# microsoft/NOTSOFAR1-Challenge

Hardware: AMD Instinct MI355X
Metric: CSS real-time-factor (sep. audio sec/wall sec) on 7-ch 16 kHz (higher is better)
Workload: dtype f32 (float32 operands on v_mfma_f32_32x32x2_f32 in every Linear layer, attention product and transform: the reference's own operand precision; MVDR covariance / solve f64)

## Files before the change

notsofar1-challenge_amd/csrc/gemm_f32.hip:

```cpp
#include <algorithm>
#include <type_traits>

#include "gemm_common.hpp"

namespace css {

namespace {

constexpr int F_BK = 16;
constexpr int F_LD = 20;
constexpr int F_BUF = (128 + BN) * F_LD;
constexpr int F_PATCH_LD = 36;

typedef float f32x4 __attribute__((ext_vector_type(4)));

__device__ __forceinline__ float epi_value(float acc, float bn, float bm, int act, bool has_res, float rv, float alpha) {
    float v = acc + bn + bm;
    if (act == ACT_RELU) v = fmaxf(v, 0.f);
    else if (act == ACT_SIGMOID) v = sigmoidf_(v);
    if (has_res) v = rv + alpha * v;
    return v;
}

template <int TM, bool BD, bool FAST>
__device__ __forceinline__ void f32_tile(const GemmArgs& g, const float* __restrict__ A, const float* __restrict__ B,
                                         float* __restrict__ C, const int m0, const int n0, float* __restrict__ lds) {
    const int tid = threadIdx.x, lane = tid & 63, w = tid >> 6, c = lane & 31, h = lane >> 5;
    const int M = g.M, N = g.N;
    constexpr int BM = 32 * TM;
    constexpr int NPA = (BM + 63) / 64;
    const int srow = tid >> 2, sk = (tid & 3) * 4;
    const int64_t extA = (int64_t)(M - 1) * g.lda + (g.lda > g.K ? g.lda : g.K), extB = (int64_t)(N - 1) * g.ldb + (g.ldb > g.K ? g.ldb : g.K);
    const __amdgpu_buffer_rsrc_t rsA = __builtin_amdgcn_make_buffer_rsrc(const_cast<float*>(A), 0, (int)(extA * 4), 0x00020000);
    const __amdgpu_buffer_rsrc_t rsB = __builtin_amdgcn_make_buffer_rsrc(const_cast<float*>(B), 0, (int)((BD ? (int64_t)((N + 31) / 32 * 32) * g.K : extB) * 4), 0x00020000);
    const int voA = (int)(((int64_t)(m0 + srow) * g.lda + sk) * 4), voB = (int)(((int64_t)(n0 + srow) * g.ldb + sk) * 4);
    const int passA = (int)(64 * g.lda * 4), passB = (int)(64 * g.ldb * 4);
    const bool a1_on = (BM % 64 == 0) || srow < BM % 64;
#ifndef F32_TOOLS
#define F32_TOOLS 0
#endif
#ifndef F32_PROBE
#define F32_PROBE 0
#endif
#ifndef F32_FAST_EPILOGUE
#define F32_FAST_EPILOGUE 1
#endif
#ifndef F32_SPREAD
#define F32_SPREAD 1
#endif
#ifndef F32_TRANSPOSED
#define F32_TRANSPOSED 0
#endif
#ifndef F32_STORE_GUARD
#define F32_STORE_GUARD 1
#endif
#if F32_STORE_GUARD
#define F32_AFTER_STORE(o) asm volatile("s_nop 0" : : "v"(o));
#else
#define F32_AFTER_STORE(o)
#endif
#ifndef F32_DMA
#define F32_DMA 0
#endif
#if F32_DMA
    constexpr int D_BUF = (128 + BN) * 16;
    const int dseg = ((tid & 3) ^ ((tid >> 4) & 3)) * 4;
    const int dvoA = (int)(((int64_t)(m0 + srow) * g.lda + dseg) * 4), dvoB = (int)(((int64_t)(n0 + srow) * g.ldb + dseg) * 4);
    const bool a1_wave = (BM % 64 == 0) || w < (BM % 64) / 16;
    typedef __attribute__((address_space(3))) void lds_void;
#define F32_GLOAD(k0, buf)                                                                                       \
    _Pragma("unroll") for (int i = 0; i < NPA; ++i) {                                                            \
        if (i + 1 < NPA || a1_wave)                                                                              \
            __builtin_amdgcn_raw_ptr_buffer_load_lds(rsA, (lds_void*)(lds + (buf) * D_BUF + (i * 64 + 16 * w) * 16), 16, dvoA, (k0) * 4 + i * passA, 0, 0); \
    }                                                                                                            \
    _Pragma("unroll") for (int i = 0; i < 2; ++i)                                                                \
        __builtin_amdgcn_raw_ptr_buffer_load_lds(rsB, (lds_void*)(lds + (buf) * D_BUF + (128 + i * 64 + 16 * w) * 16), 16, dvoB, (k0) * 4 + i * passB, 0, 0);
#define F32_LSTORE(buf) __builtin_amdgcn_s_waitcnt(0x0F70);
#define F32_GLOAD1(k0, j)
#undef F32_SPREAD
#define F32_SPREAD 0
#else
    f32x4 ra[NPA], rb[2];
    f32x4 wc[2], wn[2];
    const int vw = (int)((((int64_t)(n0 / 32 + w) * (g.K / 8)) * 64 + lane) * 16);
#define F32_GLOAD(k0, buf)                                                                                       \
    _Pragma("unroll") for (int i = 0; i < NPA; ++i) {                                                            \
        if (i + 1 < NPA || a1_on) ra[i] = __builtin_bit_cast(f32x4, __builtin_amdgcn_raw_buffer_load_b128(rsA, voA, (k0) * 4 + i * passA, 0)); \
    }                                                                                                            \
    if constexpr (!BD) {                                                                                         \
        _Pragma("unroll") for (int i = 0; i < 2; ++i)                                                            \
            rb[i] = __builtin_bit_cast(f32x4, __builtin_amdgcn_raw_buffer_load_b128(rsB, voB, (k0) * 4 + i * passB, 0)); \
    } else {                                                                                                     \
        wn[0] = __builtin_bit_cast(f32x4, __builtin_amdgcn_raw_buffer_load_b128(rsB, vw, ((k0) / 8) * 1024, 0)); \
        wn[1] = __builtin_bit_cast(f32x4, __builtin_amdgcn_raw_buffer_load_b128(rsB, vw, ((k0) / 8 + 1) * 1024, 0)); \
    }
#define F32_GLOAD1(k0, j)                                                                                        \
    {                                                                                                            \
        if ((j) < NPA) {                                                                                         \
            if ((j) + 1 < NPA || a1_on) ra[(j) < NPA ? (j) : 0] = __builtin_bit_cast(f32x4, __builtin_amdgcn_raw_buffer_load_b128(rsA, voA, (k0) * 4 + (j) * passA, 0)); \
        } else if ((j) < NPA + 2) {                                                                              \
            if constexpr (!BD) rb[(j) - NPA] = __builtin_bit_cast(f32x4, __builtin_amdgcn_raw_buffer_load_b128(rsB, voB, (k0) * 4 + ((j) - NPA) * passB, 0)); \
            else wn[(j) - NPA] = __builtin_bit_cast(f32x4, __builtin_amdgcn_raw_buffer_load_b128(rsB, vw, ((k0) / 8 + (j) - NPA) * 1024, 0)); \
        }                                                                                                        \
    }
#define F32_LSTORE(buf)                                                                                          \
    {                                                                                                            \
        float* as_ = lds + (buf) * F_BUF + srow * F_LD + sk;                                                     \
        _Pragma("unroll") for (int i = 0; i < NPA; ++i) {                                                        \
            if (i + 1 < NPA || a1_on) *reinterpret_cast<f32x4*>(as_ + i * 64 * F_LD) = ra[i];                    \
        }                                                                                                        \
        if constexpr (!BD) {                                                                                     \
            _Pragma("unroll") for (int i = 0; i < 2; ++i) *reinterpret_cast<f32x4*>(as_ + (128 + i * 64) * F_LD) = rb[i]; \
        }                                                                                                        \
    }
#endif
    f32x16 acc[TM];
#pragma unroll
    for (int i = 0; i < TM; ++i) acc[i] = f32x16{0};
    const int nk = g.K / F_BK;
#if F32_PROBE
    const unsigned long long t_in_ = (w == 0) ? __builtin_readcyclecounter() : 0;
#endif
    F32_GLOAD(0, 0)
    F32_LSTORE(0)
    if constexpr (BD) { wc[0] = wn[0]; wc[1] = wn[1]; }
    __syncthreads();
#if F32_DMA
    constexpr int S_BUF = D_BUF, S_LD = 16;
    const int sw4 = ((c >> 2) & 3) * 4;
    const int aoff = c * 16, boff = (128 + 32 * w + c) * 16;
#define F32_SLOT(ch) (((8 * (ch) + 4 * h)) ^ sw4)
#else
    constexpr int S_BUF = F_BUF, S_LD = F_LD;
    const int aoff = c * F_LD + 4 * h, boff = (128 + 32 * w + c) * F_LD + 4 * h;
#define F32_SLOT(ch) (8 * (ch))
#endif
    const float* __restrict__ bias = g.bias;
    const float* __restrict__ res = g.residual;
    const int act = g.act;
    const bool bias_m = bias && g.bias_along_m, bias_n = bias && !g.bias_along_m, has_res = res != nullptr;
    const int64_t ldc = g.ldc, ldr = g.ldr;
    const float alpha = g.alpha;
    const bool wide = FAST || ((ldc % 4 == 0) && (N % 4 == 0) && ((reinterpret_cast<uintptr_t>(C) & 15) == 0) &&
                               (!has_res || ((ldr % 4 == 0) && ((reinterpret_cast<uintptr_t>(res) & 15) == 0))));
    constexpr bool fast = FAST;
    const __amdgpu_buffer_rsrc_t rsC = __builtin_amdgcn_make_buffer_rsrc(C, 0, fast ? (int)((int64_t)M * ldc * 4) : 0, 0x00020000);
    const __amdgpu_buffer_rsrc_t rsR = __builtin_amdgcn_make_buffer_rsrc(const_cast<float*>(res), 0, (fast && has_res) ? (int)((int64_t)M * ldr * 4) : 0, 0x00020000);
    f32x4 rv[2][4];
#if F32_TRANSPOSED
    auto prefetch_fast = [&](int i, int slot, int lane_) {
        const int vo_ = (int)((((int64_t)m0 + (lane_ & 31)) * ldr + n0 + 32 * w + 4 * (lane_ >> 5)) * 4);
#pragma unroll
        for (int q = 0; q < 4; ++q)
            rv[slot][q] = __builtin_bit_cast(f32x4, __builtin_amdgcn_raw_buffer_load_b128(rsR, vo_, (int)((32 * i * ldr + 8 * q) * 4), 0));
    };
#else
    auto prefetch_fast = [&](int i, int slot, int lane_) {
        const int vo_ = (int)(((unsigned)(m0 + (lane_ >> 3)) * (unsigned)ldr + n0 + 32 * w + (lane_ & 7) * 4) * 4u);
#pragma unroll
        for (int j = 0; j < 4; ++j)
            rv[slot][j] = __builtin_bit_cast(f32x4, __builtin_amdgcn_raw_buffer_load_b128(rsR, vo_, (int)((unsigned)(32 * i + 8 * j) * (unsigned)ldr * 4u), 0));
    };
#endif
    auto prefetch = [&](int i, int slot, int lane_) {
        const int n_ = n0 + 32 * w + (lane_ & 7) * 4;
#pragma unroll
        for (int j = 0; j < 4; ++j) {
            const int m = m0 + 32 * i + (lane_ >> 3) + 8 * j;
            const int mc = m < M ? m : M - 1;
            rv[slot][j] = f32x4{0.f, 0.f, 0.f, 0.f};
            if (has_res && n_ < N) {
                if (wide) {
                    rv[slot][j] = *reinterpret_cast<const f32x4*>(res + (int64_t)mc * ldr + n_);
                } else {
#pragma unroll
                    for (int e = 0; e < 4; ++e) rv[slot][j][e] = res[(int64_t)mc * ldr + (n_ + e < N ? n_ + e : N - 1)];
                }
            }
        }
    };
#ifndef F32_ABLATE
#define F32_ABLATE 0
#endif
    f32x4 abl_a = {1.f, 2.f, 3.f, (float)lane}, abl_b = {0.5f, 0.25f, (float)w, 1.f};
#define F32_COMPUTE(buf)                                                                                         \
    {                                                                                                            \
        const float* as = lds + (buf) * S_BUF + aoff;                                                            \
        const float* bs = lds + (buf) * S_BUF + boff;                                                            \
        _Pragma("unroll") for (int ch = 0; ch < 2; ++ch) {                                                       \
            f32x4 b = abl_b;                                                                                     \
            if constexpr (BD) b = wc[ch];                                                                        \
            else if (!(F32_ABLATE & 4)) b = *reinterpret_cast<const f32x4*>(bs + F32_SLOT(ch));                  \
            f32x4 a[TM];                                                                                         \
            _Pragma("unroll") for (int i = 0; i < TM; ++i) {                                                     \
                a[i] = abl_a;                                                                                    \
                if (!(F32_ABLATE & 4)) a[i] = *reinterpret_cast<const f32x4*>(as + i * 32 * S_LD + F32_SLOT(ch)); \
            }                                                                                                    \
            __builtin_amdgcn_sched_barrier(0);                                                                   \
            _Pragma("unroll") for (int e = 0; e < 4; ++e) {                                                      \
                if (F32_SPREAD && spread_k0 >= 0 && !(e & 1)) { F32_GLOAD1(spread_k0, ch * 2 + (e >> 1)) __builtin_amdgcn_sched_barrier(0); } \
                _Pragma("unroll") for (int i = 0; i < TM; ++i) {                                                 \
                    if (F32_ABLATE & 8) asm volatile("v_mfma_f32_32x32x2_f32 %0, %1, %2, %0" : "+a"(acc[i]) : "v"(a[i][e]), "v"(b[e])); \
                    else if (F32_TRANSPOSED) acc[i] = __builtin_amdgcn_mfma_f32_32x32x2f32(b[e], a[i][e], acc[i], 0, 0, 0); \
                    else acc[i] = __builtin_amdgcn_mfma_f32_32x32x2f32(a[i][e], b[e], acc[i], 0, 0, 0);          \
                }                                                                                                \
                if (F32_SPREAD && spread_k0 >= 0) __builtin_amdgcn_sched_barrier(0);                             \
            }                                                                                                    \
            __builtin_amdgcn_sched_barrier(0);                                                                   \
        }                                                                                                        \
    }
#if F32_PROBE
    const bool probe = w == 0 && g.narrow_epilogue == 77 && g.range_flag;
    unsigned long long pc_ = 0, pl_ = 0, pb_ = 0, pt_ = 0;
    const unsigned long long t_loop_ = probe ? __builtin_readcyclecounter() : 0;
#define F32_CLK(var) if (probe) var = __builtin_readcyclecounter();
#else
#define F32_CLK(var)
#endif
    int spread_k0 = -1;
    for (int kt = 0; kt + 1 < nk; ++kt) {
#if F32_PROBE
        unsigned long long t0_ = 0, t1_ = 0, t2_ = 0, t3_ = 0;
#endif
        F32_CLK(t0_)
        if (F32_SPREAD) spread_k0 = (kt + 1) * F_BK;
        else if (!(F32_ABLATE & 2)) { F32_GLOAD((kt + 1) * F_BK, (kt + 1) & 1) }
        __builtin_amdgcn_sched_barrier(0);
        F32_COMPUTE(kt & 1)
        F32_CLK(t1_)
        if (!(F32_ABLATE & 2)) { F32_LSTORE((kt + 1) & 1) }
        if constexpr (BD) { wc[0] = wn[0]; wc[1] = wn[1]; }
        F32_CLK(t2_)
        if (!(F32_ABLATE & 1)) __syncthreads();
        F32_CLK(t3_)
#if F32_PROBE
        pc_ += t1_ - t0_; pl_ += t2_ - t1_; pb_ += t3_ - t2_; pt_ += 1;
#endif
    }
#if F32_PROBE
    if (probe && lane == 0) {
        unsigned long long* pr = reinterpret_cast<unsigned long long*>(g.range_flag) + 4096 + 4 * blockIdx.x;
        atomicAdd(pr + 0, pc_); atomicAdd(pr + 1, pl_); atomicAdd(pr + 2, pb_); atomicAdd(pr + 3, pt_);
        atomicAdd(pr + 4096 + 0, t_loop_ - t_in_);
        atomicAdd(pr + 4096 + 1, 1ull);
    }
    const unsigned long long t_out_ = probe ? __builtin_readcyclecounter() : 0;
#define F32_EPILOGUE_PROBE                                                                                       \
    if (probe && lane == 0) {                                                                                    \
        unsigned long long* pr = reinterpret_cast<unsigned long long*>(g.range_flag) + 4096 + 4 * blockIdx.x;    \
        atomicAdd(pr + 4096 + 2, __builtin_readcyclecounter() - t_out_);        \
    }
#else
#define F32_EPILOGUE_PROBE
#endif
#undef F32_CLK
    {
        int lane_ = lane;
        asm volatile("" : "+v"(lane_));
        if (fast) { if (has_res) prefetch_fast(0, 0, lane_); }
        else prefetch(0, 0, lane_);
    }
    spread_k0 = -1;
    F32_COMPUTE((nk - 1) & 1)
    __syncthreads();
#undef F32_COMPUTE
#undef F32_SLOT
#undef F32_GLOAD
#undef F32_GLOAD1
#undef F32_LSTORE

    int lane_e = lane;
    asm volatile("" : "+v"(lane_e));
    float* patch = lds + w * (32 * F_PATCH_LD);
    const int col4 = (lane_e & 7) * 4, n = n0 + 32 * w + col4, erow = lane_e >> 3;
    const bool col_ok = n < N;
    float bn[4] = {0.f, 0.f, 0.f, 0.f};
    if (bias_n) {
#pragma unroll
        for (int e = 0; e < 4; ++e) bn[e] = bias[n + e < N ? n + e : N - 1];
    }
#if F32_TRANSPOSED
    if (fast) {
        const int ce = lane_e & 31, he = lane_e >> 5, nw = n0 + 32 * w + 4 * he;
        const int voC = (int)((((int64_t)m0 + ce) * ldc + nw) * 4);
        const bool relu = act == ACT_RELU;
        f32x4 bq[4];
#pragma unroll
        for (int q = 0; q < 4; ++q) {
            bq[q] = f32x4{0.f, 0.f, 0.f, 0.f};
            if (bias_n) {
#pragma unroll
                for (int e = 0; e < 4; ++e) bq[q][e] = bias[nw + 8 * q + e];
            }
        }
#pragma unroll
        for (int i = 0; i < TM; ++i) {
            if (i + 1 < TM && has_res) prefetch_fast(i + 1, (i + 1) & 1, lane_e);
#pragma unroll
            for (int q = 0; q < 4; ++q) {
                f32x4 o;
#pragma unroll
                for (int e = 0; e < 4; ++e) {
                    float t = acc[i][4 * q + e] + bq[q][e];
                    if (relu) t = fmaxf(t, 0.f);
                    if (has_res) t = rv[i & 1][q][e] + alpha * t;
                    o[e] = t;
                }
                typedef unsigned int u32x4 __attribute__((ext_vector_type(4)));
                __builtin_amdgcn_raw_buffer_store_b128(__builtin_bit_cast(u32x4, o), rsC, voC, (int)((32 * i * ldc + 8 * q) * 4), 0);
                F32_AFTER_STORE(o)
#if F32_TRANSPOSED >= 2
                __builtin_amdgcn_sched_barrier(0);
                asm volatile("s_nop 7");
#if F32_TRANSPOSED >= 3
                asm volatile("s_nop 7");
#endif
                __builtin_amdgcn_sched_barrier(0);
#endif
            }
        }
        F32_EPILOGUE_PROBE
        return;
    }
#else
    if constexpr (FAST) {
        const int voC = (int)(((unsigned)(m0 + erow) * (unsigned)ldc + n) * 4u);
        auto epilogue = [&](auto relu_c, auto res_c) {
            const bool relu = relu_c;
            constexpr bool res = decltype(res_c)::value;
#pragma unroll
            for (int i = 0; i < TM; ++i) {
#pragma unroll
                for (int r = 0; r < 16; ++r) patch[((r & 3) + 8 * (r >> 2) + 4 * h) * F_PATCH_LD + c] = acc[i][r];
                if (i + 1 < TM && res) prefetch_fast(i + 1, (i + 1) & 1, lane_e);
#pragma unroll
                for (int j = 0; j < 4; ++j) {
                    const f32x4 v = *reinterpret_cast<const f32x4*>(patch + (erow + 8 * j) * F_PATCH_LD + col4);
                    f32x4 o;
#pragma unroll
                    for (int e = 0; e < 4; ++e) {
                        float t = v[e] + bn[e];
                        if (relu) t = fmaxf(t, 0.f);
                        if (res) t = rv[i & 1][j][e] + alpha * t;
                        o[e] = t;
                    }
                    typedef unsigned int u32x4 __attribute__((ext_vector_type(4)));
                    __builtin_amdgcn_raw_buffer_store_b128(__builtin_bit_cast(u32x4, o), rsC, voC, (int)((unsigned)(32 * i + 8 * j) * (unsigned)ldc * 4u), 0);
                    F32_AFTER_STORE(o)
                }
            }
        };
        if (has_res) epilogue(act == ACT_RELU, std::true_type{});
        else if (act == ACT_RELU) epilogue(std::true_type{}, std::false_type{});
        else epilogue(std::false_type{}, std::false_type{});
        F32_EPILOGUE_PROBE
        return;
    }
#endif
#pragma unroll
    for (int i = 0; i < TM; ++i) {
#if F32_TRANSPOSED
#pragma unroll
        for (int q = 0; q < 4; ++q)
            *reinterpret_cast<f32x4*>(patch + c * F_PATCH_LD + 8 * q + 4 * h) = f32x4{acc[i][4 * q], acc[i][4 * q + 1], acc[i][4 * q + 2], acc[i][4 * q + 3]};
#else
#pragma unroll
        for (int r = 0; r < 16; ++r) patch[((r & 3) + 8 * (r >> 2) + 4 * h) * F_PATCH_LD + c] = acc[i][r];
#endif
        if (i + 1 < TM) prefetch(i + 1, (i + 1) & 1, lane_e);
#pragma unroll
        for (int j = 0; j < 4; ++j) {
            const int row = erow + 8 * j, m = m0 + 32 * i + row;
            const f32x4 v = *reinterpret_cast<const f32x4*>(patch + row * F_PATCH_LD + col4);
            if (m >= M || !col_ok) continue;
            float* dst = C + (int64_t)m * ldc + n;
            const float bm = bias_m ? bias[m] : 0.f;
            f32x4 o;
#pragma unroll
            for (int e = 0; e < 4; ++e) o[e] = epi_value(v[e], bn[e], bm, act, has_res, rv[i & 1][j][e], alpha);
            if (wide) {
                *reinterpret_cast<f32x4*>(dst) = o;
            } else {
#pragma unroll
                for (int e = 0; e < 4; ++e)
                    if (n + e < N) dst[e] = o[e];
            }
        }
    }
    F32_EPILOGUE_PROBE
#undef F32_EPILOGUE_PROBE
}

}

struct F32Plan {
    int u, tiles_n, ncu, max_tm; int64_t U;
#if F32_TOOLS
    unsigned long long* dbg;
#endif
};

template <bool BD, bool FAST>
__global__ __launch_bounds__(256, 4) void gemm_f32_kernel(GemmArgs g, F32Plan p) {
    __shared__ __attribute__((aligned(16))) float lds[2 * F_BUF];
    const int b = blockIdx.x, v = b % p.ncu, j = b / p.ncu;
    const int64_t lo = p.U * v / p.ncu, hi = p.U * (v + 1) / p.ncu;
    int64_t pos = lo + (hi - lo) * j / 4;
    const int64_t end = lo + (hi - lo) * (j + 1) / 4;
    int want = std::min(1 + (b + j) % 4, p.max_tm);
    bool first = true;
#if F32_TOOLS
    if (p.dbg && threadIdx.x == 0) {
        p.dbg[4 * b + 0] = wall_clock64();
        p.dbg[4 * b + 2] = ((unsigned long long)__builtin_amdgcn_s_getreg(63508) << 32) | (unsigned)__builtin_amdgcn_s_getreg(63492);
        p.dbg[4 * b + 3] = __builtin_readcyclecounter();
    }
#endif
    const int64_t panel0 = pos / p.u;
    int r = (int)(pos - panel0 * p.u);
    int bz = (int)(panel0 / p.tiles_n), tn = (int)(panel0 - (int64_t)bz * p.tiles_n);
    while (pos < end) {
        const int tm = (int)std::min<int64_t>(std::min<int64_t>(want, end - pos), p.u - r);
        const float* A = g.A + (int64_t)bz * g.strideA;
        const float* B = g.B + (int64_t)bz * g.strideB;
        float* C = g.C + (int64_t)bz * g.strideC;
        if (!first) __syncthreads();
        first = false;
        switch (tm) {
            case 1: f32_tile<1, BD, FAST>(g, A, B, C, 32 * r, tn * BN, lds); break;
            case 2: f32_tile<2, BD, FAST>(g, A, B, C, 32 * r, tn * BN, lds); break;
            case 3: f32_tile<3, BD, FAST>(g, A, B, C, 32 * r, tn * BN, lds); break;
            default: f32_tile<4, BD, FAST>(g, A, B, C, 32 * r, tn * BN, lds); break;
        }
        pos += tm;
        want = p.max_tm;
        r += tm;
        if (r == p.u) {
            r = 0;
            if (++tn == p.tiles_n) { tn = 0; ++bz; }
        }
    }
#if F32_TOOLS
    if (p.dbg && threadIdx.x == 0) { p.dbg[4 * b + 1] = wall_clock64(); p.dbg[4 * b + 3] = __builtin_readcyclecounter() - p.dbg[4 * b + 3]; }
#endif
}

static bool f32_fast_epilogue(const GemmArgs& g) {
    const int64_t lim = (int64_t)1 << 31;
    const bool has_res = g.residual != nullptr;
    const bool wide = (g.ldc % 4 == 0) && (g.N % 4 == 0) && ((reinterpret_cast<uintptr_t>(g.C) & 15) == 0) &&
                      (g.batch == 1 || g.strideC % 4 == 0) &&
                      (!has_res || ((g.ldr % 4 == 0) && ((reinterpret_cast<uintptr_t>(g.residual) & 15) == 0)));
    return F32_FAST_EPILOGUE && wide && !(g.bias && g.bias_along_m) && (g.N % BN == 0) && g.act != ACT_SIGMOID &&
           (int64_t)g.M * g.ldc * 4 < lim && (!has_res || (int64_t)g.M * g.ldr * 4 < lim);
}

bool launch_gemm_f32(const GemmArgs& g, hipStream_t s, int forced_tm) {
    if (g.M <= 0 || g.N <= 0 || g.batch <= 0) return true;
    if (g.K <= 0 || g.K % F_BK) return false;
    const int64_t lim = (int64_t)1 << 31;
    if ((((int64_t)g.M + 128) * g.lda + g.K) * 4 >= lim || (((int64_t)g.N + 128) * g.ldb + g.K) * 4 >= lim) return false;
    if (g.b_frag32 && (g.N % 32 || g.K % 16 || g.batch != 1 || ((int64_t)g.N * g.K * 4 >= lim))) return false;
    if ((g.lda % 4) || (!g.b_frag32 && (g.ldb % 4)) || (reinterpret_cast<uintptr_t>(g.A) & 15) || (reinterpret_cast<uintptr_t>(g.B) & 15)) return false;
    constexpr int NCU = 256;
    F32Plan p;
    p.u = (g.M + 31) / 32;
    p.tiles_n = (g.N + BN - 1) / BN;
    p.ncu = NCU;
    p.max_tm = (forced_tm >= 1 && forced_tm <= 4) ? forced_tm : 4;
    p.U = (int64_t)p.u * p.tiles_n * g.batch;
#if F32_TOOLS
    p.dbg = g.narrow_epilogue == 77 ? reinterpret_cast<unsigned long long*>(g.range_flag) : nullptr;
#endif
    const bool fast = f32_fast_epilogue(g);
    void (*kern)(GemmArgs, F32Plan) = g.b_frag32 ? (fast ? gemm_f32_kernel<true, true> : gemm_f32_kernel<true, false>)
                                                 : (fast ? gemm_f32_kernel<false, true> : gemm_f32_kernel<false, false>);
    hipLaunchKernelGGL(kern, dim3(4 * NCU), dim3(256), 0, s, g, p);
    return true;
}


__global__ void f32_fragments_kernel(const float* __restrict__ src, int64_t ld_src, float* __restrict__ dst, int N, int K) {
    const int64_t idx = (int64_t)blockIdx.x * blockDim.x + threadIdx.x;
    const int64_t total = (int64_t)(N / 32) * (K / 8) * 64;
    if (idx >= total) return;
    const int lane = (int)(idx & 63);
    const int64_t t = idx >> 6;
    const int kc = (int)(t % (K / 8)), j = (int)(t / (K / 8));
    const float* p = src + (int64_t)(32 * j + (lane & 31)) * ld_src + 8 * kc + 4 * (lane >> 5);
    reinterpret_cast<float4*>(dst)[idx] = make_float4(p[0], p[1], p[2], p[3]);
}
void launch_f32_fragments(const float* src, int64_t ld_src, float* dst, int N, int K, hipStream_t s) {
    const int64_t total = (int64_t)(N / 32) * (K / 8) * 64;
    if (total <= 0) return;
    hipLaunchKernelGGL(f32_fragments_kernel, dim3((unsigned)((total + 255) / 256)), dim3(256), 0, s, src, ld_src, dst, N, K);
}

}
```

Baseline: 7340.

## Use deeper K slabs for fragment-weight f32 GEMM tiles with small TM

Adds a K-depth template parameter so the weights-as-fragments f32 GEMM path stages 32- or 64-wide K slabs of A in LDS for TM 1-3 tiles, instead of 16. This cuts the number of syncthreads and pipeline iterations per tile and double-buffers the A fragment reads across chunks. B fragments are prefetched per chunk inside the compute loop. It also pins some scalar arguments to SGPRs with empty asm. The cost is higher register and LDS pressure, more code size, and a reworked prefetch schedule.

```diff
diff --git a/notsofar1-challenge_amd/csrc/gemm_f32.hip b/notsofar1-challenge_amd/csrc/gemm_f32.hip
--- a/notsofar1-challenge_amd/csrc/gemm_f32.hip
+++ b/notsofar1-challenge_amd/csrc/gemm_f32.hip
@@ -22,20 +22,54 @@
     return v;
 }
 
-template <int TM, bool BD, bool FAST>
+#ifndef F32_DMA
+#define F32_DMA 0
+#endif
+#ifndef F32_SPREAD
+#define F32_SPREAD 1
+#endif
+#ifndef F32_DEEP
+#define F32_DEEP 1
+#endif
+#ifndef F32_DEEP_TM1
+#define F32_DEEP_TM1 64
+#endif
+#ifndef F32_DEEP_TM2
+#define F32_DEEP_TM2 32
+#endif
+#ifndef F32_DEEP_TM3
+#define F32_DEEP_TM3 32
+#endif
+constexpr int f32_max_depth(int tm, bool bd) {
+    return (!bd || !F32_DEEP || !F32_SPREAD || F32_DMA) ? 16 : tm == 1 ? F32_DEEP_TM1 : tm == 2 ? F32_DEEP_TM2 : tm == 3 ? F32_DEEP_TM3 : 16;
+}
+
+template <int TM, bool BD, bool FAST, int DK>
 __device__ __forceinline__ void f32_tile(const GemmArgs& g, const float* __restrict__ A, const float* __restrict__ B,
                                          float* __restrict__ C, const int m0, const int n0, float* __restrict__ lds) {
-    const int tid = threadIdx.x, lane = tid & 63, w = tid >> 6, c = lane & 31, h = lane >> 5;
+    int tid = threadIdx.x;
+    asm volatile("" : "+v"(tid));
+    const int lane = tid & 63, w = tid >> 6, c = lane & 31, h = lane >> 5;
     const int M = g.M, N = g.N;
+    int gK = g.K;
+    int64_t glda = g.lda;
+    if constexpr (FAST) asm volatile("" : "+s"(gK), "+s"(glda));
     constexpr int BM = 32 * TM;
-    constexpr int NPA = (BM + 63) / 64;
-    const int srow = tid >> 2, sk = (tid & 3) * 4;
-    const int64_t extA = (int64_t)(M - 1) * g.lda + (g.lda > g.K ? g.lda : g.K), extB = (int64_t)(N - 1) * g.ldb + (g.ldb > g.K ? g.ldb : g.K);
+    constexpr int LD = DK + 4;
+    constexpr int PPR = DK / 4;
+    constexpr int RPP = 256 / PPR;
+    constexpr int NPA = (BM + RPP - 1) / RPP;
+    constexpr int NCH = DK / 8;
+    static_assert(DK == 16 || (BD && (DK == 32 || DK == 64)), "deep slabs: the weights-as-fragments kernels only");
+    static_assert(BM * LD <= (BD ? F_BUF : 128 * F_LD), "the A slab must fit its buffer");
+    static_assert(!F32_DMA || DK == 16, "the DMA path stages 16-float rows");
+    const int srow = tid / PPR, sk = (tid % PPR) * 4;
+    const int64_t extA = (int64_t)(M - 1) * glda + (glda > gK ? glda : gK), extB = (int64_t)(N - 1) * g.ldb + (g.ldb > gK ? g.ldb : gK);
     const __amdgpu_buffer_rsrc_t rsA = __builtin_amdgcn_make_buffer_rsrc(const_cast<float*>(A), 0, (int)(extA * 4), 0x00020000);
-    const __amdgpu_buffer_rsrc_t rsB = __builtin_amdgcn_make_buffer_rsrc(const_cast<float*>(B), 0, (int)((BD ? (int64_t)((N + 31) / 32 * 32) * g.K : extB) * 4), 0x00020000);
-    const int voA = (int)(((int64_t)(m0 + srow) * g.lda + sk) * 4), voB = (int)(((int64_t)(n0 + srow) * g.ldb + sk) * 4);
-    const int passA = (int)(64 * g.lda * 4), passB = (int)(64 * g.ldb * 4);
-    const bool a1_on = (BM % 64 == 0) || srow < BM % 64;
+    const __amdgpu_buffer_rsrc_t rsB = __builtin_amdgcn_make_buffer_rsrc(const_cast<float*>(B), 0, (int)((BD ? (int64_t)((N + 31) / 32 * 32) * gK : extB) * 4), 0x00020000);
+    const int voA = (int)(((int64_t)(m0 + srow) * glda + sk) * 4), voB = (int)(((int64_t)(n0 + srow) * g.ldb + sk) * 4);
+    const int passA = (int)(RPP * glda * 4), passB = (int)(64 * g.ldb * 4);
+    const bool a1_on = (BM % RPP == 0) || srow < BM % RPP;
 #ifndef F32_TOOLS
 #define F32_TOOLS 0
 #endif
@@ -45,9 +79,6 @@
 #ifndef F32_FAST_EPILOGUE
 #define F32_FAST_EPILOGUE 1
 #endif
-#ifndef F32_SPREAD
-#define F32_SPREAD 1
-#endif
 #ifndef F32_TRANSPOSED
 #define F32_TRANSPOSED 0
 #endif
@@ -59,13 +90,12 @@
 #else
 #define F32_AFTER_STORE(o)
 #endif
-#ifndef F32_DMA
-#define F32_DMA 0
-#endif
 #if F32_DMA
     constexpr int D_BUF = (128 + BN) * 16;
+    f32x4 wc[NCH] = {}, wn[NCH] = {};
+    const int vw = 0;
     const int dseg = ((tid & 3) ^ ((tid >> 4) & 3)) * 4;
-    const int dvoA = (int)(((int64_t)(m0 + srow) * g.lda + dseg) * 4), dvoB = (int)(((int64_t)(n0 + srow) * g.ldb + dseg) * 4);
+    const int dvoA = (int)(((int64_t)(m0 + srow) * glda + dseg) * 4), dvoB = (int)(((int64_t)(n0 + srow) * g.ldb + dseg) * 4);
     const bool a1_wave = (BM % 64 == 0) || w < (BM % 64) / 16;
     typedef __attribute__((address_space(3))) void lds_void;
 #define F32_GLOAD(k0, buf)                                                                                       \
@@ -81,8 +111,8 @@
 #define F32_SPREAD 0
 #else
     f32x4 ra[NPA], rb[2];
-    f32x4 wc[2], wn[2];
-    const int vw = (int)((((int64_t)(n0 / 32 + w) * (g.K / 8)) * 64 + lane) * 16);
+    f32x4 wc[NCH], wn[DK == 16 ? NCH : 1];
+    const int vw = (int)((((int64_t)(n0 / 32 + w) * (gK / 8)) * 64 + lane) * 16);
 #define F32_GLOAD(k0, buf)                                                                                       \
     _Pragma("unroll") for (int i = 0; i < NPA; ++i) {                                                            \
         if (i + 1 < NPA || a1_on) ra[i] = __builtin_bit_cast(f32x4, __builtin_amdgcn_raw_buffer_load_b128(rsA, voA, (k0) * 4 + i * passA, 0)); \
@@ -91,39 +121,41 @@
         _Pragma("unroll") for (int i = 0; i < 2; ++i)                                                            \
             rb[i] = __builtin_bit_cast(f32x4, __builtin_amdgcn_raw_buffer_load_b128(rsB, voB, (k0) * 4 + i * passB, 0)); \
     } else {                                                                                                     \
-        wn[0] = __builtin_bit_cast(f32x4, __builtin_amdgcn_raw_buffer_load_b128(rsB, vw, ((k0) / 8) * 1024, 0)); \
-        wn[1] = __builtin_bit_cast(f32x4, __builtin_amdgcn_raw_buffer_load_b128(rsB, vw, ((k0) / 8 + 1) * 1024, 0)); \
+        _Pragma("unroll") for (int i = 0; i < (DK == 16 ? NCH : NCH - 1); ++i) {    \
+            const f32x4 w_ = __builtin_bit_cast(f32x4, __builtin_amdgcn_raw_buffer_load_b128(rsB, vw, ((k0) / 8 + i) * 1024, 0)); \
+            if constexpr (DK == 16) wn[i] = w_; else wc[i] = w_;                                                 \
+        }                                                                                                        \
     }
 #define F32_GLOAD1(k0, j)                                                                                        \
     {                                                                                                            \
         if ((j) < NPA) {                                                                                         \
             if ((j) + 1 < NPA || a1_on) ra[(j) < NPA ? (j) : 0] = __builtin_bit_cast(f32x4, __builtin_amdgcn_raw_buffer_load_b128(rsA, voA, (k0) * 4 + (j) * passA, 0)); \
-        } else if ((j) < NPA + 2) {                                                                              \
-            if constexpr (!BD) rb[(j) - NPA] = __builtin_bit_cast(f32x4, __builtin_amdgcn_raw_buffer_load_b128(rsB, voB, (k0) * 4 + ((j) - NPA) * passB, 0)); \
-            else wn[(j) - NPA] = __builtin_bit_cast(f32x4, __builtin_amdgcn_raw_buffer_load_b128(rsB, vw, ((k0) / 8 + (j) - NPA) * 1024, 0)); \
+        } else if ((j) < NPA + (BD ? NCH : 2)) {                                                                 \
+            if constexpr (!BD) rb[((j) - NPA) & 1] = __builtin_bit_cast(f32x4, __builtin_amdgcn_raw_buffer_load_b128(rsB, voB, (k0) * 4 + ((j) - NPA) * passB, 0)); \
+            else wn[DK == 16 ? ((j) - NPA) & 1 : 0] = __builtin_bit_cast(f32x4, __builtin_amdgcn_raw_buffer_load_b128(rsB, vw, ((k0) / 8 + (j) - NPA) * 1024, 0)); \
         }                                                                                                        \
     }
 #define F32_LSTORE(buf)                                                                                          \
     {                                                                                                            \
-        float* as_ = lds + (buf) * F_BUF + srow * F_LD + sk;                                                     \
+        float* as_ = lds + (buf) * F_BUF + srow * LD + sk;                                                       \
         _Pragma("unroll") for (int i = 0; i < NPA; ++i) {                                                        \
-            if (i + 1 < NPA || a1_on) *reinterpret_cast<f32x4*>(as_ + i * 64 * F_LD) = ra[i];                    \
+            if (i + 1 < NPA || a1_on) *reinterpret_cast<f32x4*>(as_ + i * RPP * LD) = ra[i];                     \
         }                                                                                                        \
         if constexpr (!BD) {                                                                                     \
-            _Pragma("unroll") for (int i = 0; i < 2; ++i) *reinterpret_cast<f32x4*>(as_ + (128 + i * 64) * F_LD) = rb[i]; \
+            _Pragma("unroll") for (int i = 0; i < 2; ++i) *reinterpret_cast<f32x4*>(as_ + (128 + i * 64) * LD) = rb[i]; \
         }                                                                                                        \
     }
 #endif
     f32x16 acc[TM];
 #pragma unroll
     for (int i = 0; i < TM; ++i) acc[i] = f32x16{0};
-    const int nk = g.K / F_BK;
+    const int nk = gK / DK;
 #if F32_PROBE
     const unsigned long long t_in_ = (w == 0) ? __builtin_readcyclecounter() : 0;
 #endif
     F32_GLOAD(0, 0)
     F32_LSTORE(0)
-    if constexpr (BD) { wc[0] = wn[0]; wc[1] = wn[1]; }
+    if constexpr (BD && DK == 16) { wc[0] = wn[0]; wc[1] = wn[1]; }
     __syncthreads();
 #if F32_DMA
     constexpr int S_BUF = D_BUF, S_LD = 16;
@@ -131,15 +163,16 @@
     const int aoff = c * 16, boff = (128 + 32 * w + c) * 16;
 #define F32_SLOT(ch) (((8 * (ch) + 4 * h)) ^ sw4)
 #else
-    constexpr int S_BUF = F_BUF, S_LD = F_LD;
-    const int aoff = c * F_LD + 4 * h, boff = (128 + 32 * w + c) * F_LD + 4 * h;
+    constexpr int S_BUF = F_BUF, S_LD = LD;
+    const int aoff = c * LD + 4 * h, boff = (128 + 32 * w + c) * LD + 4 * h;
 #define F32_SLOT(ch) (8 * (ch))
 #endif
     const float* __restrict__ bias = g.bias;
     const float* __restrict__ res = g.residual;
     const int act = g.act;
     const bool bias_m = bias && g.bias_along_m, bias_n = bias && !g.bias_along_m, has_res = res != nullptr;
-    const int64_t ldc = g.ldc, ldr = g.ldr;
+    int64_t ldc = g.ldc, ldr = g.ldr;
+    if constexpr (FAST) asm volatile("" : "+s"(ldc), "+s"(ldr));
     const float alpha = g.alpha;
     const bool wide = FAST || ((ldc % 4 == 0) && (N % 4 == 0) && ((reinterpret_cast<uintptr_t>(C) & 15) == 0) &&
                                (!has_res || ((ldr % 4 == 0) && ((reinterpret_cast<uintptr_t>(res) & 15) == 0))));
@@ -183,30 +216,59 @@
 #define F32_ABLATE 0
 #endif
     f32x4 abl_a = {1.f, 2.f, 3.f, (float)lane}, abl_b = {0.5f, 0.25f, (float)w, 1.f};
+#define F32_MFMA(i, av, bv)                                                                                      \
+    {                                                                                                            \
+        if (F32_ABLATE & 8) asm volatile("v_mfma_f32_32x32x2_f32 %0, %1, %2, %0" : "+a"(acc[i]) : "v"(av), "v"(bv)); \
+        else if (F32_TRANSPOSED) acc[i] = __builtin_amdgcn_mfma_f32_32x32x2f32(bv, av, acc[i], 0, 0, 0);         \
+        else acc[i] = __builtin_amdgcn_mfma_f32_32x32x2f32(av, bv, acc[i], 0, 0, 0);                             \
+    }
 #define F32_COMPUTE(buf)                                                                                         \
     {                                                                                                            \
         const float* as = lds + (buf) * S_BUF + aoff;                                                            \
         const float* bs = lds + (buf) * S_BUF + boff;                                                            \
-        _Pragma("unroll") for (int ch = 0; ch < 2; ++ch) {                                                       \
-            f32x4 b = abl_b;                                                                                     \
-            if constexpr (BD) b = wc[ch];                                                                        \
-            else if (!(F32_ABLATE & 4)) b = *reinterpret_cast<const f32x4*>(bs + F32_SLOT(ch));                  \
-            f32x4 a[TM];                                                                                         \
+        if constexpr (DK == 16) {                                                                                \
+            _Pragma("unroll") for (int ch = 0; ch < 2; ++ch) {                                                   \
+                f32x4 b = abl_b;                                                                                 \
+                if constexpr (BD) b = wc[ch];                                                                    \
+                else if (!(F32_ABLATE & 4)) b = *reinterpret_cast<const f32x4*>(bs + F32_SLOT(ch));              \
+                f32x4 a[TM];                                                                                     \
+                _Pragma("unroll") for (int i = 0; i < TM; ++i) {                                                 \
+                    a[i] = abl_a;                                                                                \
+                    if (!(F32_ABLATE & 4)) a[i] = *reinterpret_cast<const f32x4*>(as + i * 32 * S_LD + F32_SLOT(ch)); \
+                }                                                                                                \
+                __builtin_amdgcn_sched_barrier(0);                                                               \
+                _Pragma("unroll") for (int e = 0; e < 4; ++e) {                                                  \
+                    if (F32_SPREAD && spread_k0 >= 0 && !(e & 1)) { F32_GLOAD1(spread_k0, ch * 2 + (e >> 1)) __builtin_amdgcn_sched_barrier(0); } \
+                    _Pragma("unroll") for (int i = 0; i < TM; ++i) F32_MFMA(i, a[i][e], b[e])                    \
+                    if (F32_SPREAD && spread_k0 >= 0) __builtin_amdgcn_sched_barrier(0);                         \
+                }                                                                                                \
+                __builtin_amdgcn_sched_barrier(0);                                                               \
+            }                                                                                                    \
+        } else {                                                                                                 \
+            wc[NCH - 1] = __builtin_bit_cast(f32x4, __builtin_amdgcn_raw_buffer_load_b128(rsB, vw, (cur_k0 / 8 + NCH - 1) * 1024, 0)); \
+            f32x4 a[2][TM];                                                                                      \
             _Pragma("unroll") for (int i = 0; i < TM; ++i) {                                                     \
-                a[i] = abl_a;                                                                                    \
-                if (!(F32_ABLATE & 4)) a[i] = *reinterpret_cast<const f32x4*>(as + i * 32 * S_LD + F32_SLOT(ch)); \
+                a[0][i] = abl_a;                                                                                 \
+                if (!(F32_ABLATE & 4)) a[0][i] = *reinterpret_cast<const f32x4*>(as + i * 32 * S_LD);            \
             }                                                                                                    \
-            __builtin_amdgcn_sched_barrier(0);                                                                   \
-            _Pragma("unroll") for (int e = 0; e < 4; ++e) {                                                      \
-                if (F32_SPREAD && spread_k0 >= 0 && !(e & 1)) { F32_GLOAD1(spread_k0, ch * 2 + (e >> 1)) __builtin_amdgcn_sched_barrier(0); } \
-                _Pragma("unroll") for (int i = 0; i < TM; ++i) {                                                 \
-                    if (F32_ABLATE & 8) asm volatile("v_mfma_f32_32x32x2_f32 %0, %1, %2, %0" : "+a"(acc[i]) : "v"(a[i][e]), "v"(b[e])); \
-                    else if (F32_TRANSPOSED) acc[i] = __builtin_amdgcn_mfma_f32_32x32x2f32(b[e], a[i][e], acc[i], 0, 0, 0); \
-                    else acc[i] = __builtin_amdgcn_mfma_f32_32x32x2f32(a[i][e], b[e], acc[i], 0, 0, 0);          \
+            _Pragma("unroll") for (int ch = 0; ch < NCH; ++ch) {                                                 \
+                if (ch + 1 < NCH) {                                                                              \
+                    _Pragma("unroll") for (int i = 0; i < TM; ++i) {                                             \
+                        a[(ch + 1) & 1][i] = abl_a;                                                              \
+                        if (!(F32_ABLATE & 4)) a[(ch + 1) & 1][i] = *reinterpret_cast<const f32x4*>(as + i * 32 * S_LD + 8 * (ch + 1)); \
+                    }                                                                                            \
                 }                                                                                                \
-                if (F32_SPREAD && spread_k0 >= 0) __builtin_amdgcn_sched_barrier(0);                             \
+                __builtin_amdgcn_sched_barrier(0);                                                               \
+                _Pragma("unroll") for (int e = 0; e < 4; ++e) {                                                  \
+                    if (spread_k0 >= 0 && ch * 4 + e < NPA) { F32_GLOAD1(spread_k0, ch * 4 + e) __builtin_amdgcn_sched_barrier(0); } \
+                    _Pragma("unroll") for (int i = 0; i < TM; ++i) F32_MFMA(i, a[ch & 1][i][e], wc[ch][e])       \
+                    if (spread_k0 >= 0) __builtin_amdgcn_sched_barrier(0);                                       \
+                }                                                                                                \
+                if (spread_k0 >= 0 && ch + 1 < NCH) {                                                            \
+                    wc[ch] = __builtin_bit_cast(f32x4, __builtin_amdgcn_raw_buffer_load_b128(rsB, vw, (spread_k0 / 8 + ch) * 1024, 0)); \
+                }                                                                                                \
+                __builtin_amdgcn_sched_barrier(0);                                                               \
             }                                                                                                    \
-            __builtin_amdgcn_sched_barrier(0);                                                                   \
         }                                                                                                        \
     }
 #if F32_PROBE
@@ -217,19 +279,20 @@
 #else
 #define F32_CLK(var)
 #endif
-    int spread_k0 = -1;
+    int spread_k0 = -1, cur_k0 = 0;
     for (int kt = 0; kt + 1 < nk; ++kt) {
 #if F32_PROBE
         unsigned long long t0_ = 0, t1_ = 0, t2_ = 0, t3_ = 0;
 #endif
         F32_CLK(t0_)
-        if (F32_SPREAD) spread_k0 = (kt + 1) * F_BK;
-        else if (!(F32_ABLATE & 2)) { F32_GLOAD((kt + 1) * F_BK, (kt + 1) & 1) }
+        cur_k0 = kt * DK;
+        if (F32_SPREAD) spread_k0 = (kt + 1) * DK;
+        else if (!(F32_ABLATE & 2)) { F32_GLOAD((kt + 1) * DK, (kt + 1) & 1) }
         __builtin_amdgcn_sched_barrier(0);
         F32_COMPUTE(kt & 1)
         F32_CLK(t1_)
         if (!(F32_ABLATE & 2)) { F32_LSTORE((kt + 1) & 1) }
-        if constexpr (BD) { wc[0] = wn[0]; wc[1] = wn[1]; }
+        if constexpr (BD && DK == 16) { wc[0] = wn[0]; wc[1] = wn[1]; }
         F32_CLK(t2_)
         if (!(F32_ABLATE & 1)) __syncthreads();
         F32_CLK(t3_)
@@ -261,9 +324,11 @@
         else prefetch(0, 0, lane_);
     }
     spread_k0 = -1;
+    cur_k0 = (nk - 1) * DK;
     F32_COMPUTE((nk - 1) & 1)
     __syncthreads();
 #undef F32_COMPUTE
+#undef F32_MFMA
 #undef F32_SLOT
 #undef F32_GLOAD
 #undef F32_GLOAD1
@@ -391,6 +456,19 @@
 #undef F32_EPILOGUE_PROBE
 }
 
+template <int TM, bool BD, bool FAST>
+__device__ __forceinline__ void f32_tile_any(const GemmArgs& g, const float* __restrict__ A, const float* __restrict__ B,
+                                             float* __restrict__ C, const int m0, const int n0, float* __restrict__ lds) {
+    constexpr int D = f32_max_depth(TM, BD && FAST);
+    if constexpr (D >= 64) {
+        if (g.K % 64 == 0) return f32_tile<TM, BD, FAST, 64>(g, A, B, C, m0, n0, lds);
+    }
+    if constexpr (D >= 32) {
+        if (g.K % 32 == 0) return f32_tile<TM, BD, FAST, 32>(g, A, B, C, m0, n0, lds);
+    }
+    f32_tile<TM, BD, FAST, 16>(g, A, B, C, m0, n0, lds);
+}
+
 }
 
 struct F32Plan {
@@ -427,10 +505,10 @@
         if (!first) __syncthreads();
         first = false;
         switch (tm) {
-            case 1: f32_tile<1, BD, FAST>(g, A, B, C, 32 * r, tn * BN, lds); break;
-            case 2: f32_tile<2, BD, FAST>(g, A, B, C, 32 * r, tn * BN, lds); break;
-            case 3: f32_tile<3, BD, FAST>(g, A, B, C, 32 * r, tn * BN, lds); break;
-            default: f32_tile<4, BD, FAST>(g, A, B, C, 32 * r, tn * BN, lds); break;
+            case 1: f32_tile_any<1, BD, FAST>(g, A, B, C, 32 * r, tn * BN, lds); break;
+            case 2: f32_tile_any<2, BD, FAST>(g, A, B, C, 32 * r, tn * BN, lds); break;
+            case 3: f32_tile_any<3, BD, FAST>(g, A, B, C, 32 * r, tn * BN, lds); break;
+            default: f32_tile_any<4, BD, FAST>(g, A, B, C, 32 * r, tn * BN, lds); break;
         }
         pos += tm;
         want = p.max_tm;
@@ -460,6 +538,9 @@
     if (g.K <= 0 || g.K % F_BK) return false;
     const int64_t lim = (int64_t)1 << 31;
     if ((((int64_t)g.M + 128) * g.lda + g.K) * 4 >= lim || (((int64_t)g.N + 128) * g.ldb + g.K) * 4 >= lim) return false;
+#if F32_DMA
+    if (g.b_frag32) return false;
+#endif
     if (g.b_frag32 && (g.N % 32 || g.K % 16 || g.batch != 1 || ((int64_t)g.N * g.K * 4 >= lim))) return false;
     if ((g.lda % 4) || (!g.b_frag32 && (g.ldb % 4)) || (reinterpret_cast<uintptr_t>(g.A) & 15) || (reinterpret_cast<uintptr_t>(g.B) & 15)) return false;
     constexpr int NCU = 256;
```

After: 7433, median of 6. +1.3%, better.
